# Bob-cheng/DepthModelHardening

Hardware: AMD Instinct MI355X
Metric: adv-train images/sec @1024x320, 10-step PGD, bs32 (higher is better)
Workload: dtype f32; 1 GPU; Monodepth2 ResNet18 1024x320, 10-step PGD-L_inf attack on 12 scenes, train batch 32/GPU, stereo photometric+SSIM+smoothness loss (md2), Adam; config_index=2, global_batch=32, per_gpu_batch=32, parallelism=dp1, attack_overlap=False, attack_scenes=12, graph_attack=False

## Files before the change

### depthmodelhardening_amd/csrc/down_conv.hip

```cpp
#include "common.hpp"

using namespace dmh;

namespace {

typedef float f32x16 __attribute__((ext_vector_type(16)));

constexpr int NT = 256;
constexpr int TR = 4, TC = 32;
constexpr int CK = 8, NPAIR = CK / 2;
constexpr unsigned OOB = 0x80000000u;

constexpr int A_PITCH = 36;
constexpr int A_ELEMS = 64 * 2 * A_PITCH;
constexpr int A_NW = A_ELEMS / NT;
constexpr int D_ELEMS = 64 * 2 * NPAIR;
constexpr int D_NW = D_ELEMS / NT;

template <int NW, int ND>
__device__ __forceinline__ void filter_offsets(int tid, int r0, int inner, unsigned (&wo)[NW], unsigned (&dofs)[ND]) {
#pragma unroll
    for (int i = 0; i < NW; ++i) {
        const int d = tid + i * NT, rowh = d / A_PITCH, q = d - rowh * A_PITCH;
        const int row = rowh >> 1, hh = rowh & 1, t = q >> 2, p = q & 3;
        wo[i] = (unsigned)(((r0 + row) * inner + 2 * p + hh) * 9 + t) * 4u;
    }
#pragma unroll
    for (int i = 0; i < ND; ++i) {
        const int d = tid + i * NT, rowh = d >> 2, p = d & 3;
        dofs[i] = (unsigned)((r0 + (rowh >> 1)) * inner + 2 * p + (rowh & 1)) * 4u;
    }
}

typedef float f32x4 __attribute__((ext_vector_type(4)));
constexpr int IMG_A = 32 * 2 * A_PITCH;
constexpr int IMG_D = 32 * 2 * NPAIR;
constexpr int IMG_G = IMG_A + IMG_D;
constexpr int IMG_WORDS = IMG_G / 4;
constexpr int IMG_NW = (IMG_WORDS + NT - 1) / NT;

__global__ __launch_bounds__(NT) void down_weight_image_kernel(const float* __restrict__ w3, const float* __restrict__ wd, int rows,
                                                               int inner, float* __restrict__ img) {
    const size_t idx = (size_t)blockIdx.x * NT + threadIdx.x;
    const int nch = inner / CK;
    if (idx >= (size_t)(rows / 32) * nch * IMG_G) return;
    const int e = (int)(idx % IMG_G);
    const int gc = (int)(idx / IMG_G), rg = gc / nch, ch = gc - rg * nch;
    float v;
    if (e < IMG_A) {
        const int rowh = e / A_PITCH, q = e - rowh * A_PITCH, t = q >> 2, p = q & 3;
        v = w3[((size_t)(rg * 32 + (rowh >> 1)) * inner + ch * CK + 2 * p + (rowh & 1)) * 9 + t];
    } else {
        const int d = e - IMG_A, rowh = d >> 2, p = d & 3;
        v = wd ? wd[(size_t)(rg * 32 + (rowh >> 1)) * inner + ch * CK + 2 * p + (rowh & 1)] : 0.f;
    }
    img[idx] = v;
}

__device__ __forceinline__ f32x4 ldb4(rsrc_t rs, unsigned byte_off, unsigned s_off) {
    return __builtin_bit_cast(f32x4, __builtin_amdgcn_raw_buffer_load_b128(rs, byte_off, s_off, 0));
}

constexpr int F_PR = 3 * TR, F_PC = 2 * TC + 1, F_PEL = F_PR * F_PC, F_PLANE = F_PEL + 1;
constexpr int F_NP = (CK * F_PEL + NT - 1) / NT;

struct FArgs {
    const float *x, *w3, *wd;
    const float *shift3, *shiftd;
    int relu3;
    float *y3, *yd;
    int B, Cin, Cout, H, W, Ho, Wo, gx, gy, gk;
};

template <bool DOWN>
__device__ __forceinline__ void fwd_store(const FArgs& a, const f32x16& accA, const f32x16& accB, const f32x16& accDA,
                                          const f32x16& accDB, int R, int ox, int h, int k0, int NR) {
    const int b = R / a.Ho, oy = R - b * a.Ho;
    if (R < NR && ox < a.Wo) {
        const size_t HWo = (size_t)a.Ho * a.Wo;
        const size_t o = ((size_t)b * a.Cout + k0) * HWo + (size_t)oy * a.Wo + ox;
#pragma unroll
        for (int v = 0; v < 16; ++v) {
            const int i = 8 * (v >> 2) + 4 * h + (v & 3);
            float ya = accA[v], yb = accB[v];
            if (a.shift3) {
                ya += a.shift3[k0 + i];
                yb += a.shift3[k0 + i + 32];
            }
            if (a.relu3) {
                ya = fmaxf(ya, 0.f);
                yb = fmaxf(yb, 0.f);
            }
            a.y3[o + (size_t)i * HWo] = ya;
            a.y3[o + (size_t)(i + 32) * HWo] = yb;
            if constexpr (DOWN) {
                float da = accDA[v], db = accDB[v];
                if (a.shiftd) {
                    da += a.shiftd[k0 + i];
                    db += a.shiftd[k0 + i + 32];
                }
                a.yd[o + (size_t)i * HWo] = da;
                a.yd[o + (size_t)(i + 32) * HWo] = db;
            }
        }
    }
}

template <bool DOWN>
__global__ __launch_bounds__(NT, 2) void down_conv_fwd_kernel(const FArgs a) {
    __shared__ float patch[CK * F_PLANE];
    __shared__ __attribute__((aligned(16))) float wt[A_ELEMS];
    __shared__ __attribute__((aligned(16))) float wdl[D_ELEMS];
    const int tid = threadIdx.x, lane = tid & 63, wv = tid >> 6, n = lane & 31, h = lane >> 5;
    int q = blockIdx.x;
    const int kt = q % a.gk;
    q /= a.gk;
    const int bxi = q % a.gx, rt = q / a.gx;
    const int R0 = rt * TR, ox0 = bxi * TC, k0 = kt * 64;
    const int ix0 = 2 * ox0 - 1, NR = a.B * a.Ho;
    const unsigned HW = (unsigned)(a.H * a.W);
    const rsrc_t rx = make_rsrc(a.x, (unsigned)a.B * (unsigned)a.Cin * HW * 4u);
    const rsrc_t rw = make_rsrc(a.w3, (unsigned)a.Cout * (unsigned)a.Cin * 36u);
    const rsrc_t rd = make_rsrc(DOWN ? a.wd : a.w3, (unsigned)a.Cout * (unsigned)a.Cin * 4u);

    unsigned po[F_NP], wo[A_NW], dofs[D_NW];
#pragma unroll
    for (int i = 0; i < F_NP; ++i) {
        const int e = tid + i * NT, c = e / F_PEL, rem = e - c * F_PEL, r = rem / F_PC, cc = rem - r * F_PC;
        const int R = R0 + r / 3, bb = R / a.Ho, oy = R - bb * a.Ho;
        const int iy = 2 * oy - 1 + r % 3, ix = ix0 + cc;
        const bool ok = e < CK * F_PEL && R < NR && iy >= 0 && iy < a.H && ix >= 0 && ix < a.W;
        po[i] = ok ? ((unsigned)(bb * a.Cin + c) * HW + (unsigned)(iy * a.W + ix)) * 4u : OOB;
    }
    filter_offsets(tid, k0, a.Cin, wo, dofs);

    float rp[F_NP], rwv[A_NW], rdv[D_NW];
    auto fetch = [&](const int c0) __attribute__((always_inline)) {
        const unsigned sp = (unsigned)c0 * HW * 4u, sw = (unsigned)c0 * 36u, sd = (unsigned)c0 * 4u;
#pragma unroll
        for (int i = 0; i < F_NP; ++i) rp[i] = ldb(rx, po[i], sp);
#pragma unroll
        for (int i = 0; i < A_NW; ++i) rwv[i] = ldb(rw, wo[i], sw);
        if constexpr (DOWN) {
#pragma unroll
            for (int i = 0; i < D_NW; ++i) rdv[i] = ldb(rd, dofs[i], sd);
        }
    };
    auto commit = [&]() __attribute__((always_inline)) {
#pragma unroll
        for (int i = 0; i < F_NP; ++i) {
            const int e = tid + i * NT;
            if (i < F_NP - 1 || e < CK * F_PEL) patch[e + e / F_PEL] = rp[i];
        }
#pragma unroll
        for (int i = 0; i < A_NW; ++i) wt[tid + i * NT] = rwv[i];
        if constexpr (DOWN) {
#pragma unroll
            for (int i = 0; i < D_NW; ++i) wdl[tid + i * NT] = rdv[i];
        }
    };

    f32x16 accA, accB, accDA, accDB;
#pragma unroll
    for (int v = 0; v < 16; ++v) accA[v] = accB[v] = accDA[v] = accDB[v] = 0.f;
    const float* pb = patch + h * F_PLANE + (3 * wv) * F_PC + 2 * n;
    const float* aA = wt + (n * 2 + h) * A_PITCH;
    const float* aB = aA + 32 * 2 * A_PITCH;
    const float* dA = wdl + (n * 2 + h) * NPAIR;
    const float* dB = dA + 32 * 2 * NPAIR;

    const int chunks = a.Cin / CK;
    fetch(0);
    for (int ch = 0; ch < chunks; ++ch) {
        __syncthreads();
        commit();
        __syncthreads();
        if (ch + 1 < chunks) fetch((ch + 1) * CK);
        float4 da = make_float4(0.f, 0.f, 0.f, 0.f), db = da;
        if constexpr (DOWN) {
            da = *reinterpret_cast<const float4*>(dA);
            db = *reinterpret_cast<const float4*>(dB);
        }
#pragma unroll
        for (int t = 0; t < 9; ++t) {
            const float4 wa = *reinterpret_cast<const float4*>(aA + 4 * t);
            const float4 wb = *reinterpret_cast<const float4*>(aB + 4 * t);
            const float was[4] = {wa.x, wa.y, wa.z, wa.w}, wbs[4] = {wb.x, wb.y, wb.z, wb.w};
            const float das[4] = {da.x, da.y, da.z, da.w}, dbs[4] = {db.x, db.y, db.z, db.w};
#pragma unroll
            for (int p = 0; p < NPAIR; ++p) {
                const float bv = pb[2 * p * F_PLANE + (t / 3) * F_PC + (t % 3)];
                accA = __builtin_amdgcn_mfma_f32_32x32x2f32(was[p], bv, accA, 0, 0, 0);
                accB = __builtin_amdgcn_mfma_f32_32x32x2f32(wbs[p], bv, accB, 0, 0, 0);
                if (DOWN && t == 4) {
                    accDA = __builtin_amdgcn_mfma_f32_32x32x2f32(das[p], bv, accDA, 0, 0, 0);
                    accDB = __builtin_amdgcn_mfma_f32_32x32x2f32(dbs[p], bv, accDB, 0, 0, 0);
                }
            }
        }
    }
    fwd_store<DOWN>(a, accA, accB, accDA, accDB, R0 + wv, ox0 + n, h, k0, NR);
}

constexpr int FW_WPR = 17, FW_SUB = 2 * FW_WPR, FW_ROW = 2 * FW_SUB;
constexpr int FW_PLANE = 864;
constexpr int FW_NWORD = CK * F_PR * FW_WPR;
constexpr int FW_NP = (FW_NWORD + NT - 1) / NT;
static_assert(FW_PLANE >= F_PR * FW_ROW && FW_PLANE % 64 == 32, "plane pitch");

template <bool DOWN>
__global__ __launch_bounds__(NT, 2) void down_conv_fwd_wide_kernel(const FArgs a) {
    __shared__ __attribute__((aligned(16))) float patch[CK * FW_PLANE];
    __shared__ f32x4 wimg[2 * IMG_WORDS];
    const int tid = threadIdx.x, lane = tid & 63, wv = tid >> 6, n = lane & 31, h = lane >> 5;
    int q = blockIdx.x;
    const int kt = q % a.gk;
    q /= a.gk;
    const int bxi = q % a.gx, rt = q / a.gx;
    const int R0 = rt * TR, ox0 = bxi * TC, k0 = kt * 64;
    const int NR = a.B * a.Ho, nch = a.Cin / CK;
    const unsigned HW = (unsigned)(a.H * a.W);
    const rsrc_t rx = make_rsrc(a.x, (unsigned)a.B * (unsigned)a.Cin * HW * 4u);
    const rsrc_t ri = make_rsrc(a.w3, (unsigned)(a.Cout / 32) * (unsigned)nch * (unsigned)(IMG_G * 4));

    unsigned po[FW_NP];
    int lo[FW_NP];
#pragma unroll
    for (int i = 0; i < FW_NP; ++i) {
        const int e = tid + i * NT, c = e / (F_PR * FW_WPR), rem = e - c * (F_PR * FW_WPR), r = rem / FW_WPR, w = rem - r * FW_WPR;
        const int R = R0 + r / 3, bb = R / a.Ho, oy = R - bb * a.Ho;
        const int iy = 2 * oy - 1 + r % 3, ix = 2 * ox0 - 4 + 4 * w;
        const bool ok = e < FW_NWORD && R < NR && iy >= 0 && iy < a.H && ix >= 0 && ix < a.W;
        po[i] = ok ? ((unsigned)(bb * a.Cin + c) * HW + (unsigned)(iy * a.W + ix)) * 4u : OOB;
        lo[i] = c * FW_PLANE + r * FW_ROW + 2 * w;
    }
    const unsigned wofs = (unsigned)tid * 16u;
    const unsigned gstep = (unsigned)nch * (unsigned)(IMG_G * 4);
    const unsigned g0 = (unsigned)(2 * kt) * gstep;

    f32x4 rp[FW_NP], rw[2 * IMG_NW];
    auto fetch = [&](const int ch) __attribute__((always_inline)) {
        const unsigned sp = (unsigned)(ch * CK) * HW * 4u;
#pragma unroll
        for (int i = 0; i < FW_NP; ++i) rp[i] = ldb4(rx, po[i], sp);
        const unsigned sw = g0 + (unsigned)ch * (unsigned)(IMG_G * 4);
#pragma unroll
        for (int g = 0; g < 2; ++g)
#pragma unroll
            for (int j = 0; j < IMG_NW; ++j)
                rw[g * IMG_NW + j] = ldb4(ri, ((j + 1) * NT <= IMG_WORDS || j * NT + tid < IMG_WORDS) ? wofs + (unsigned)(j * NT * 16) : OOB,
                                          sw + (unsigned)g * gstep);
    };
    auto commit = [&]() __attribute__((always_inline)) {
#pragma unroll
        for (int i = 0; i < FW_NP; ++i) {
            if (i < FW_NP - 1 || tid + i * NT < FW_NWORD) {
                *reinterpret_cast<float2*>(patch + lo[i]) = make_float2(rp[i][0], rp[i][2]);
                *reinterpret_cast<float2*>(patch + lo[i] + FW_SUB) = make_float2(rp[i][1], rp[i][3]);
            }
        }
#pragma unroll
        for (int g = 0; g < 2; ++g)
#pragma unroll
            for (int j = 0; j < IMG_NW; ++j)
                if ((j + 1) * NT <= IMG_WORDS || j * NT + tid < IMG_WORDS) wimg[g * IMG_WORDS + j * NT + tid] = rw[g * IMG_NW + j];
    };

    f32x16 accA, accB, accDA, accDB;
#pragma unroll
    for (int v = 0; v < 16; ++v) accA[v] = accB[v] = accDA[v] = accDB[v] = 0.f;
    const float* pb = patch + h * FW_PLANE + (3 * wv) * FW_ROW + n;
    const float* wf = reinterpret_cast<const float*>(wimg);
    const float* aA = wf + (n * 2 + h) * A_PITCH;
    const float* aB = aA + IMG_G;
    const float* dA = wf + IMG_A + (n * 2 + h) * NPAIR;
    const float* dB = dA + IMG_G;

    fetch(0);
    for (int ch = 0; ch < nch; ++ch) {
        __syncthreads();
        commit();
        __syncthreads();
        if (ch + 1 < nch) fetch(ch + 1);
        float4 da = make_float4(0.f, 0.f, 0.f, 0.f), db = da;
        if constexpr (DOWN) {
            da = *reinterpret_cast<const float4*>(dA);
            db = *reinterpret_cast<const float4*>(dB);
        }
#pragma unroll
        for (int t = 0; t < 9; ++t) {
            const float4 wa = *reinterpret_cast<const float4*>(aA + 4 * t);
            const float4 wb = *reinterpret_cast<const float4*>(aB + 4 * t);
            const float was[4] = {wa.x, wa.y, wa.z, wa.w}, wbs[4] = {wb.x, wb.y, wb.z, wb.w};
            const float das[4] = {da.x, da.y, da.z, da.w}, dbs[4] = {db.x, db.y, db.z, db.w};
            const int kx = t % 3, off = (t / 3) * FW_ROW + (kx == 1 ? 2 : FW_SUB + (kx == 0 ? 1 : 2));
#pragma unroll
            for (int p = 0; p < NPAIR; ++p) {
                const float bv = pb[2 * p * FW_PLANE + off];
                accA = __builtin_amdgcn_mfma_f32_32x32x2f32(was[p], bv, accA, 0, 0, 0);
                accB = __builtin_amdgcn_mfma_f32_32x32x2f32(wbs[p], bv, accB, 0, 0, 0);
                if (DOWN && t == 4) {
                    accDA = __builtin_amdgcn_mfma_f32_32x32x2f32(das[p], bv, accDA, 0, 0, 0);
                    accDB = __builtin_amdgcn_mfma_f32_32x32x2f32(dbs[p], bv, accDB, 0, 0, 0);
                }
            }
        }
    }
    fwd_store<DOWN>(a, accA, accB, accDA, accDB, R0 + wv, ox0 + n, h, k0, NR);
}

constexpr int B_PR = 2 * TR, B_PC = TC + 1, B_PEL = B_PR * B_PC, B_PLANE = B_PEL + 1;
constexpr int B_NP = (CK * B_PEL + NT - 1) / NT;
constexpr int G_PLANE = TR * TC + 1;
constexpr int G_NP = CK * TR * TC / NT;

struct BArgs {
    const float *g3, *gd, *w3t, *wdt;
    const float* gadd;
    float* gx;
    int B, Cin, Cout, H, W, Ho, Wo, tx, ty, gc;
};

template <int MH>
__device__ __forceinline__ void bwd_store(const BArgs& a, const f32x16 (&acc)[4][MH], int R, int bc, int h, int c0m, int NR) {
    const int b = R / a.Ho, ar = R - b * a.Ho;
    if (R < NR && bc < a.Wo) {
        const size_t HW = (size_t)a.H * a.W;
        const size_t o = ((size_t)b * a.Cin + c0m) * HW + (size_t)(2 * ar) * a.W + 2 * bc;
#pragma unroll
        for (int half = 0; half < MH; ++half)
#pragma unroll
            for (int v = 0; v < 16; ++v) {
                const int i = 8 * (v >> 2) + 4 * h + (v & 3) + 32 * half;
                float* g = a.gx + o + (size_t)i * HW;
                float2 r0 = make_float2(acc[0][half][v], acc[1][half][v]), r1 = make_float2(acc[2][half][v], acc[3][half][v]);
                if (a.gadd) {
                    const float* q = a.gadd + o + (size_t)i * HW;
                    const float2 q0 = *reinterpret_cast<const float2*>(q), q1 = *reinterpret_cast<const float2*>(q + a.W);
                    r0.x += q0.x; r0.y += q0.y; r1.x += q1.x; r1.y += q1.y;
                }
                *reinterpret_cast<float2*>(g) = r0;
                *reinterpret_cast<float2*>(g + a.W) = r1;
            }
    }
}

template <bool DOWN, int MH>
__global__ __launch_bounds__(NT, 2) void down_conv_bwd_kernel(const BArgs a) {
    constexpr int W_NW = A_NW * MH / 2, W_ND = D_NW * MH / 2;
    __shared__ float patch[CK * B_PLANE];
    __shared__ float gdl[CK * G_PLANE];
    __shared__ __attribute__((aligned(16))) float wt[A_ELEMS * MH / 2];
    __shared__ __attribute__((aligned(16))) float wdl[D_ELEMS * MH / 2];
    const int tid = threadIdx.x, lane = tid & 63, wv = tid >> 6, n = lane & 31, h = lane >> 5;
    int q = blockIdx.x;
    const int ct = q % a.gc;
    q /= a.gc;
    const int bxi = q % a.tx, rt = q / a.tx;
    const int R0 = rt * TR, b0 = bxi * TC, c0m = ct * 32 * MH, NR = a.B * a.Ho;
    const unsigned HWo = (unsigned)(a.Ho * a.Wo);
    const rsrc_t rg = make_rsrc(a.g3, (unsigned)a.B * (unsigned)a.Cout * HWo * 4u);
    const rsrc_t rgd = make_rsrc(DOWN ? a.gd : a.g3, (unsigned)a.B * (unsigned)a.Cout * HWo * 4u);
    const rsrc_t rw = make_rsrc(a.w3t, (unsigned)a.Cout * (unsigned)a.Cin * 36u);
    const rsrc_t rd = make_rsrc(DOWN ? a.wdt : a.w3t, (unsigned)a.Cout * (unsigned)a.Cin * 4u);

    unsigned po[B_NP], go[G_NP], wo[W_NW], dofs[W_ND];
#pragma unroll
    for (int i = 0; i < B_NP; ++i) {
        const int e = tid + i * NT, c = e / B_PEL, rem = e - c * B_PEL, r = rem / B_PC, cc = rem - r * B_PC;
        const int R = R0 + (r >> 1), bb = R / a.Ho, oy = R - bb * a.Ho + (r & 1), ox = b0 + cc;
        const bool ok = e < CK * B_PEL && R < NR && oy < a.Ho && ox < a.Wo;
        po[i] = ok ? ((unsigned)(bb * a.Cout + c) * HWo + (unsigned)(oy * a.Wo + ox)) * 4u : OOB;
    }
#pragma unroll
    for (int i = 0; i < G_NP; ++i) {
        const int e = tid + i * NT, c = e / (TR * TC), rem = e - c * (TR * TC), r = rem / TC, cc = rem - r * TC;
        const int R = R0 + r, bb = R / a.Ho, oy = R - bb * a.Ho, ox = b0 + cc;
        go[i] = (R < NR && ox < a.Wo) ? ((unsigned)(bb * a.Cout + c) * HWo + (unsigned)(oy * a.Wo + ox)) * 4u : OOB;
    }
    filter_offsets(tid, c0m, a.Cout, wo, dofs);

    float rp[B_NP], rg4[G_NP], rwv[W_NW], rdv[W_ND];
    auto fetch = [&](const int k0) __attribute__((always_inline)) {
        const unsigned sp = (unsigned)k0 * HWo * 4u, sw = (unsigned)k0 * 36u, sd = (unsigned)k0 * 4u;
#pragma unroll
        for (int i = 0; i < B_NP; ++i) rp[i] = ldb(rg, po[i], sp);
#pragma unroll
        for (int i = 0; i < W_NW; ++i) rwv[i] = ldb(rw, wo[i], sw);
        if constexpr (DOWN) {
#pragma unroll
            for (int i = 0; i < G_NP; ++i) rg4[i] = ldb(rgd, go[i], sp);
#pragma unroll
            for (int i = 0; i < W_ND; ++i) rdv[i] = ldb(rd, dofs[i], sd);
        }
    };
    auto commit = [&]() __attribute__((always_inline)) {
#pragma unroll
        for (int i = 0; i < B_NP; ++i) {
            const int e = tid + i * NT;
            if (i < B_NP - 1 || e < CK * B_PEL) patch[e + e / B_PEL] = rp[i];
        }
#pragma unroll
        for (int i = 0; i < W_NW; ++i) wt[tid + i * NT] = rwv[i];
        if constexpr (DOWN) {
#pragma unroll
            for (int i = 0; i < G_NP; ++i) {
                const int e = tid + i * NT, c = e / (TR * TC);
                gdl[e + c] = rg4[i];
            }
#pragma unroll
            for (int i = 0; i < W_ND; ++i) wdl[tid + i * NT] = rdv[i];
        }
    };

    f32x16 acc[4][MH];
#pragma unroll
    for (int c = 0; c < 4; ++c)
#pragma unroll
        for (int m = 0; m < MH; ++m)
#pragma unroll
            for (int v = 0; v < 16; ++v) acc[c][m][v] = 0.f;
    const float* pg = patch + h * B_PLANE + (2 * wv) * B_PC + n;
    const float* pd = gdl + h * G_PLANE + wv * TC + n;
    const float* aA = wt + (n * 2 + h) * A_PITCH;
    const float* aB = aA + 32 * 2 * A_PITCH;
    const float* dA = wdl + (n * 2 + h) * NPAIR;
    const float* dB = dA + 32 * 2 * NPAIR;

    const int chunks = a.Cout / CK;
    fetch(0);
    for (int ch = 0; ch < chunks; ++ch) {
        __syncthreads();
        commit();
        __syncthreads();
        if (ch + 1 < chunks) fetch((ch + 1) * CK);
        float bv[NPAIR][2][2];
#pragma unroll
        for (int p = 0; p < NPAIR; ++p) {
            bv[p][0][0] = pg[2 * p * B_PLANE];
            bv[p][0][1] = pg[2 * p * B_PLANE + 1];
            bv[p][1][0] = pg[2 * p * B_PLANE + B_PC];
            bv[p][1][1] = pg[2 * p * B_PLANE + B_PC + 1];
        }
#pragma unroll
        for (int t = 0; t < 9; ++t) {
            const int ky = t / 3, kx = t % 3;
            const int cls = 2 * (ky != 1 ? 1 : 0) + (kx != 1 ? 1 : 0), dy = ky == 0 ? 1 : 0, dx = kx == 0 ? 1 : 0;
            const float4 wa = *reinterpret_cast<const float4*>(aA + 4 * t);
            const float4 wb = *reinterpret_cast<const float4*>((MH == 2 ? aB : aA) + 4 * t);
            const float was[4] = {wa.x, wa.y, wa.z, wa.w}, wbs[4] = {wb.x, wb.y, wb.z, wb.w};
#pragma unroll
            for (int p = 0; p < NPAIR; ++p) {
                acc[cls][0] = __builtin_amdgcn_mfma_f32_32x32x2f32(was[p], bv[p][dy][dx], acc[cls][0], 0, 0, 0);
                if constexpr (MH == 2)
                    acc[cls][1] = __builtin_amdgcn_mfma_f32_32x32x2f32(wbs[p], bv[p][dy][dx], acc[cls][1], 0, 0, 0);
            }
        }
        if constexpr (DOWN) {
            const float4 da = *reinterpret_cast<const float4*>(dA), db = *reinterpret_cast<const float4*>(MH == 2 ? dB : dA);
            const float das[4] = {da.x, da.y, da.z, da.w}, dbs[4] = {db.x, db.y, db.z, db.w};
#pragma unroll
            for (int p = 0; p < NPAIR; ++p) {
                const float gv = pd[2 * p * G_PLANE];
                acc[0][0] = __builtin_amdgcn_mfma_f32_32x32x2f32(das[p], gv, acc[0][0], 0, 0, 0);
                if constexpr (MH == 2) acc[0][1] = __builtin_amdgcn_mfma_f32_32x32x2f32(dbs[p], gv, acc[0][1], 0, 0, 0);
            }
        }
    }
    bwd_store<MH>(a, acc, R0 + wv, b0 + n, h, c0m, NR);
}

constexpr int BW_WPR = 9, BW_ROW = 4 * BW_WPR, BW_PLANE = B_PR * BW_ROW;
constexpr int BW_NWORD = CK * B_PR * BW_WPR;
constexpr int BW_NP = (BW_NWORD + NT - 1) / NT;
constexpr int GW_PLANE = 160;
static_assert(BW_PLANE % 64 == 32 && GW_PLANE % 64 == 32 && CK * TR * (TC / 4) == NT, "wide backward layout");

template <bool DOWN, int MH>
__global__ __launch_bounds__(NT, 2) void down_conv_bwd_wide_kernel(const BArgs a) {
    __shared__ f32x4 patch4[CK * BW_PLANE / 4];
    __shared__ f32x4 gdl4[CK * GW_PLANE / 4];
    __shared__ f32x4 wimg[MH * IMG_WORDS];
    const int tid = threadIdx.x, lane = tid & 63, wv = tid >> 6, n = lane & 31, h = lane >> 5;
    int q = blockIdx.x;
    const int ct = q % a.gc;
    q /= a.gc;
    const int bxi = q % a.tx, rt = q / a.tx;
    const int R0 = rt * TR, b0 = bxi * TC, c0m = ct * 32 * MH, NR = a.B * a.Ho, nch = a.Cout / CK;
    const unsigned HWo = (unsigned)(a.Ho * a.Wo);
    const rsrc_t rg = make_rsrc(a.g3, (unsigned)a.B * (unsigned)a.Cout * HWo * 4u);
    const rsrc_t rgd = make_rsrc(DOWN ? a.gd : a.g3, (unsigned)a.B * (unsigned)a.Cout * HWo * 4u);
    const rsrc_t ri = make_rsrc(a.w3t, (unsigned)(a.Cin / 32) * (unsigned)nch * (unsigned)(IMG_G * 4));

    unsigned po[BW_NP], go;
#pragma unroll
    for (int i = 0; i < BW_NP; ++i) {
        const int e = tid + i * NT, c = e / (B_PR * BW_WPR), rem = e - c * (B_PR * BW_WPR), r = rem / BW_WPR, w = rem - r * BW_WPR;
        const int R = R0 + (r >> 1), bb = R / a.Ho, oy = R - bb * a.Ho + (r & 1), ox = b0 + 4 * w;
        const bool ok = e < BW_NWORD && R < NR && oy < a.Ho && ox < a.Wo;
        po[i] = ok ? ((unsigned)(bb * a.Cout + c) * HWo + (unsigned)(oy * a.Wo + ox)) * 4u : OOB;
    }
    {
        const int c = tid / (TR * (TC / 4)), rem = tid - c * (TR * (TC / 4)), r = rem / (TC / 4), w = rem - r * (TC / 4);
        const int R = R0 + r, bb = R / a.Ho, oy = R - bb * a.Ho, ox = b0 + 4 * w;
        go = (R < NR && ox < a.Wo) ? ((unsigned)(bb * a.Cout + c) * HWo + (unsigned)(oy * a.Wo + ox)) * 4u : OOB;
    }
    const int gslot = (tid / (TR * (TC / 4))) * (GW_PLANE / 4) + (tid % (TR * (TC / 4)));
    const unsigned wofs = (unsigned)tid * 16u;
    const unsigned gstep = (unsigned)nch * (unsigned)(IMG_G * 4);
    const unsigned g0 = (unsigned)(ct * MH) * gstep;

    f32x4 rp[BW_NP], rg4, rw[MH * IMG_NW];
    auto fetch = [&](const int ch) __attribute__((always_inline)) {
        const unsigned sp = (unsigned)(ch * CK) * HWo * 4u;
#pragma unroll
        for (int i = 0; i < BW_NP; ++i) rp[i] = ldb4(rg, po[i], sp);
        if constexpr (DOWN) rg4 = ldb4(rgd, go, sp);
        const unsigned sw = g0 + (unsigned)ch * (unsigned)(IMG_G * 4);
#pragma unroll
        for (int g = 0; g < MH; ++g)
#pragma unroll
            for (int j = 0; j < IMG_NW; ++j)
                rw[g * IMG_NW + j] = ldb4(ri, ((j + 1) * NT <= IMG_WORDS || j * NT + tid < IMG_WORDS) ? wofs + (unsigned)(j * NT * 16) : OOB,
                                          sw + (unsigned)g * gstep);
    };
    auto commit = [&]() __attribute__((always_inline)) {
#pragma unroll
        for (int i = 0; i < BW_NP; ++i)
            if ((i + 1) * NT <= BW_NWORD || tid + i * NT < BW_NWORD) patch4[tid + i * NT] = rp[i];
        if constexpr (DOWN) gdl4[gslot] = rg4;
#pragma unroll
        for (int g = 0; g < MH; ++g)
#pragma unroll
            for (int j = 0; j < IMG_NW; ++j)
                if ((j + 1) * NT <= IMG_WORDS || j * NT + tid < IMG_WORDS) wimg[g * IMG_WORDS + j * NT + tid] = rw[g * IMG_NW + j];
    };

    f32x16 acc[4][MH];
#pragma unroll
    for (int c = 0; c < 4; ++c)
#pragma unroll
        for (int m = 0; m < MH; ++m)
#pragma unroll
            for (int v = 0; v < 16; ++v) acc[c][m][v] = 0.f;
    const float* pg = reinterpret_cast<const float*>(patch4) + h * BW_PLANE + (2 * wv) * BW_ROW + n;
    const float* pd = reinterpret_cast<const float*>(gdl4) + h * GW_PLANE + wv * TC + n;
    const float* wf = reinterpret_cast<const float*>(wimg);
    const float* aA = wf + (n * 2 + h) * A_PITCH;
    const float* aB = aA + (MH == 2 ? IMG_G : 0);
    const float* dA = wf + IMG_A + (n * 2 + h) * NPAIR;
    const float* dB = dA + (MH == 2 ? IMG_G : 0);

    fetch(0);
    for (int ch = 0; ch < nch; ++ch) {
        __syncthreads();
        commit();
        __syncthreads();
        if (ch + 1 < nch) fetch(ch + 1);
        float bv[NPAIR][2][2];
#pragma unroll
        for (int p = 0; p < NPAIR; ++p) {
            bv[p][0][0] = pg[2 * p * BW_PLANE];
            bv[p][0][1] = pg[2 * p * BW_PLANE + 1];
            bv[p][1][0] = pg[2 * p * BW_PLANE + BW_ROW];
            bv[p][1][1] = pg[2 * p * BW_PLANE + BW_ROW + 1];
        }
#pragma unroll
        for (int t = 0; t < 9; ++t) {
            const int ky = t / 3, kx = t % 3;
            const int cls = 2 * (ky != 1 ? 1 : 0) + (kx != 1 ? 1 : 0), dy = ky == 0 ? 1 : 0, dx = kx == 0 ? 1 : 0;
            const float4 wa = *reinterpret_cast<const float4*>(aA + 4 * t);
            const float4 wb = *reinterpret_cast<const float4*>(aB + 4 * t);
            const float was[4] = {wa.x, wa.y, wa.z, wa.w}, wbs[4] = {wb.x, wb.y, wb.z, wb.w};
#pragma unroll
            for (int p = 0; p < NPAIR; ++p) {
                acc[cls][0] = __builtin_amdgcn_mfma_f32_32x32x2f32(was[p], bv[p][dy][dx], acc[cls][0], 0, 0, 0);
                if constexpr (MH == 2)
                    acc[cls][1] = __builtin_amdgcn_mfma_f32_32x32x2f32(wbs[p], bv[p][dy][dx], acc[cls][1], 0, 0, 0);
            }
        }
        if constexpr (DOWN) {
            const float4 da = *reinterpret_cast<const float4*>(dA), db = *reinterpret_cast<const float4*>(dB);
            const float das[4] = {da.x, da.y, da.z, da.w}, dbs[4] = {db.x, db.y, db.z, db.w};
#pragma unroll
            for (int p = 0; p < NPAIR; ++p) {
                const float gv = pd[2 * p * GW_PLANE];
                acc[0][0] = __builtin_amdgcn_mfma_f32_32x32x2f32(das[p], gv, acc[0][0], 0, 0, 0);
                if constexpr (MH == 2) acc[0][1] = __builtin_amdgcn_mfma_f32_32x32x2f32(dbs[p], gv, acc[0][1], 0, 0, 0);
            }
        }
    }
    bwd_store<MH>(a, acc, R0 + wv, b0 + n, h, c0m, NR);
}

int check_sizes(int B, int Cin, int Cout, int H, int W) {
    DMH_REQUIRE(B > 0 && Cin > 0 && Cout > 0 && H >= 2 && W >= 2 && (H & 1) == 0 && (W & 1) == 0,
                "input height and width must be even");
    const int64_t cmax = Cin > Cout ? Cin : Cout;
    DMH_REQUIRE((int64_t)B * cmax * H * W < ((int64_t)1 << 29) && (int64_t)Cin * Cout < ((int64_t)1 << 24),
                "tensor too large (32-bit byte offsets)");
    return DMH_OK;
}

}

extern "C" {

int dmh_down_conv_fwd_act(const float* x, const float* w3, const float* wd, const float* shift3, const float* shiftd,
                          int relu3, int B, int Cin, int Cout, int H, int W, float* y3, float* yd, void* stream);

int dmh_down_conv_fwd(const float* x, const float* w3, const float* wd, int B, int Cin, int Cout, int H, int W,
                      float* y3, float* yd, void* stream) {
    return dmh_down_conv_fwd_act(x, w3, wd, nullptr, nullptr, 0, B, Cin, Cout, H, W, y3, yd, stream);
}

int dmh_down_conv_fwd_act(const float* x, const float* w3, const float* wd, const float* shift3, const float* shiftd,
                          int relu3, int B, int Cin, int Cout, int H, int W, float* y3, float* yd, void* stream) {
    DMH_REQUIRE(x && w3 && y3 && ((wd == nullptr) == (yd == nullptr)), "null pointer");
    DMH_REQUIRE(shiftd == nullptr || wd != nullptr, "shiftd without the shortcut convolution");
    if (int rc = check_sizes(B, Cin, Cout, H, W)) return rc;
    DMH_REQUIRE(Cin % CK == 0 && Cout % 64 == 0, "C_in must be a multiple of 8 and C_out of 64");
    FArgs a;
    a.x = x;
    a.w3 = w3;
    a.wd = wd;
    a.shift3 = shift3;
    a.shiftd = shiftd;
    a.relu3 = relu3 ? 1 : 0;
    a.y3 = y3;
    a.yd = yd;
    a.B = B;
    a.Cin = Cin;
    a.Cout = Cout;
    a.H = H;
    a.W = W;
    a.Ho = H / 2;
    a.Wo = W / 2;
    a.gx = (a.Wo + TC - 1) / TC;
    a.gy = (B * a.Ho + TR - 1) / TR;
    a.gk = Cout / 64;
    const long long blocks = (long long)a.gx * a.gy * a.gk;
    DMH_REQUIRE(blocks < (1ll << 31), "grid too large");
    if (wd)
        hipLaunchKernelGGL(down_conv_fwd_kernel<true>, dim3((unsigned)blocks), dim3(NT), 0, (hipStream_t)stream, a);
    else
        hipLaunchKernelGGL(down_conv_fwd_kernel<false>, dim3((unsigned)blocks), dim3(NT), 0, (hipStream_t)stream, a);
    return check_launch("dmh_down_conv_fwd_act");
}

int64_t dmh_down_conv_image_size(int rows, int inner) {
    if (rows <= 0 || inner <= 0 || rows % 32 || inner % CK) return -1;
    return (int64_t)(rows / 32) * (inner / CK) * IMG_G;
}

int dmh_down_conv_weight_image(const float* w3, const float* wd, int rows, int inner, float* image, void* stream) {
    DMH_REQUIRE(w3 && image, "null pointer");
    const int64_t n = dmh_down_conv_image_size(rows, inner);
    DMH_REQUIRE(n > 0 && n < ((int64_t)1 << 29), "rows must be a multiple of 32 and inner of 8");
    hipLaunchKernelGGL(down_weight_image_kernel, dim3((unsigned)((n + NT - 1) / NT)), dim3(NT), 0, (hipStream_t)stream, w3, wd, rows,
                       inner, image);
    return check_launch("dmh_down_conv_weight_image");
}

int dmh_down_conv_fwd_img(const float* x, const float* image, int has_down, const float* shift3, const float* shiftd, int relu3,
                          int B, int Cin, int Cout, int H, int W, float* y3, float* yd, void* stream) {
    DMH_REQUIRE(x && image && y3 && ((has_down != 0) == (yd != nullptr)), "null pointer");
    DMH_REQUIRE(shiftd == nullptr || has_down, "shiftd without the shortcut convolution");
    if (int rc = check_sizes(B, Cin, Cout, H, W)) return rc;
    DMH_REQUIRE(Cin % CK == 0 && Cout % 64 == 0, "C_in must be a multiple of 8 and C_out of 64");
    DMH_REQUIRE(W % 4 == 0, "the image form reads 16-byte words: W must be a multiple of 4 (use dmh_down_conv_fwd_act otherwise)");
    FArgs a;
    a.x = x;
    a.w3 = image;
    a.wd = has_down ? image : nullptr;
    a.shift3 = shift3;
    a.shiftd = shiftd;
    a.relu3 = relu3 ? 1 : 0;
    a.y3 = y3;
    a.yd = yd;
    a.B = B;
    a.Cin = Cin;
    a.Cout = Cout;
    a.H = H;
    a.W = W;
    a.Ho = H / 2;
    a.Wo = W / 2;
    a.gx = (a.Wo + TC - 1) / TC;
    a.gy = (B * a.Ho + TR - 1) / TR;
    a.gk = Cout / 64;
    const long long blocks = (long long)a.gx * a.gy * a.gk;
    DMH_REQUIRE(blocks < (1ll << 31), "grid too large");
    if (has_down)
        hipLaunchKernelGGL(down_conv_fwd_wide_kernel<true>, dim3((unsigned)blocks), dim3(NT), 0, (hipStream_t)stream, a);
    else
        hipLaunchKernelGGL(down_conv_fwd_wide_kernel<false>, dim3((unsigned)blocks), dim3(NT), 0, (hipStream_t)stream, a);
    return check_launch("dmh_down_conv_fwd_img");
}

int dmh_down_conv_bwd_data(const float* g3, const float* gd, const float* w3t, const float* wdt, int B, int Cin, int Cout,
                           int H, int W, float* g_x, void* stream) {
    return dmh_down_conv_bwd_data_acc(g3, gd, w3t, wdt, nullptr, B, Cin, Cout, H, W, g_x, stream);
}

int dmh_down_conv_bwd_data_acc(const float* g3, const float* gd, const float* w3t, const float* wdt, const float* g_add, int B,
                               int Cin, int Cout, int H, int W, float* g_x, void* stream) {
    DMH_REQUIRE(g3 && w3t && g_x && ((gd == nullptr) == (wdt == nullptr)), "null pointer");
    if (int rc = check_sizes(B, Cin, Cout, H, W)) return rc;
    DMH_REQUIRE(Cout % CK == 0 && Cin % 64 == 0, "C_out must be a multiple of 8 and C_in of 64");
    const long long tiles = (long long)((W / 2 + TC - 1) / TC) * ((B * (H / 2) + TR - 1) / TR);
    const int mh = tiles * (Cin / 64) < 200 ? 1 : 2;
    BArgs a;
    a.g3 = g3;
    a.gd = gd;
    a.w3t = w3t;
    a.wdt = wdt;
    a.gadd = g_add;
    a.gx = g_x;
    a.B = B;
    a.Cin = Cin;
    a.Cout = Cout;
    a.H = H;
    a.W = W;
    a.Ho = H / 2;
    a.Wo = W / 2;
    a.tx = (a.Wo + TC - 1) / TC;
    a.ty = (B * a.Ho + TR - 1) / TR;
    a.gc = Cin / (32 * mh);
    const long long blocks = (long long)a.tx * a.ty * a.gc;
    DMH_REQUIRE(blocks < (1ll << 31), "grid too large");
    if (gd && mh == 2)
        hipLaunchKernelGGL((down_conv_bwd_kernel<true, 2>), dim3((unsigned)blocks), dim3(NT), 0, (hipStream_t)stream, a);
    else if (gd)
        hipLaunchKernelGGL((down_conv_bwd_kernel<true, 1>), dim3((unsigned)blocks), dim3(NT), 0, (hipStream_t)stream, a);
    else if (mh == 2)
        hipLaunchKernelGGL((down_conv_bwd_kernel<false, 2>), dim3((unsigned)blocks), dim3(NT), 0, (hipStream_t)stream, a);
    else
        hipLaunchKernelGGL((down_conv_bwd_kernel<false, 1>), dim3((unsigned)blocks), dim3(NT), 0, (hipStream_t)stream, a);
    return check_launch("dmh_down_conv_bwd_data");
}

int dmh_down_conv_bwd_data_img(const float* g3, const float* gd, const float* image, const float* g_add, int B, int Cin, int Cout,
                               int H, int W, float* g_x, void* stream) {
    DMH_REQUIRE(g3 && image && g_x, "null pointer");
    if (int rc = check_sizes(B, Cin, Cout, H, W)) return rc;
    DMH_REQUIRE(Cout % CK == 0 && Cin % 64 == 0, "C_out must be a multiple of 8 and C_in of 64");
    DMH_REQUIRE(W % 8 == 0, "the image form reads 16-byte words: W must be a multiple of 8 (use dmh_down_conv_bwd_data_acc otherwise)");
    const long long tiles = (long long)((W / 2 + TC - 1) / TC) * ((B * (H / 2) + TR - 1) / TR);
    const int mh = tiles * (Cin / 64) < 200 ? 1 : 2;
    BArgs a;
    a.g3 = g3;
    a.gd = gd;
    a.w3t = image;
    a.wdt = gd ? image : nullptr;
    a.gadd = g_add;
    a.gx = g_x;
    a.B = B;
    a.Cin = Cin;
    a.Cout = Cout;
    a.H = H;
    a.W = W;
    a.Ho = H / 2;
    a.Wo = W / 2;
    a.tx = (a.Wo + TC - 1) / TC;
    a.ty = (B * a.Ho + TR - 1) / TR;
    a.gc = Cin / (32 * mh);
    const long long blocks = (long long)a.tx * a.ty * a.gc;
    DMH_REQUIRE(blocks < (1ll << 31), "grid too large");
    if (gd && mh == 2)
        hipLaunchKernelGGL((down_conv_bwd_wide_kernel<true, 2>), dim3((unsigned)blocks), dim3(NT), 0, (hipStream_t)stream, a);
    else if (gd)
        hipLaunchKernelGGL((down_conv_bwd_wide_kernel<true, 1>), dim3((unsigned)blocks), dim3(NT), 0, (hipStream_t)stream, a);
    else if (mh == 2)
        hipLaunchKernelGGL((down_conv_bwd_wide_kernel<false, 2>), dim3((unsigned)blocks), dim3(NT), 0, (hipStream_t)stream, a);
    else
        hipLaunchKernelGGL((down_conv_bwd_wide_kernel<false, 1>), dim3((unsigned)blocks), dim3(NT), 0, (hipStream_t)stream, a);
    return check_launch("dmh_down_conv_bwd_data_img");
}

}
```

Baseline: 405.6 images/s.

## Add double-buffered LDS pipelined kernels for strided down-conv forward and backward

Adds new forward and backward-data kernels for the stride-2 down convolution that double-buffer input tiles and weight images in dynamic LDS. The global loads for chunk ch+2 are interleaved with the MFMA issue of chunk ch under explicit scheduling barriers, so memory latency is hidden behind compute. The forward pipe kernel is used only when the grid fits within one wave of CUs, while the backward pipe kernel is always used. The larger LDS footprint may reduce occupancy, and the register staging adds pressure.

```diff
diff --git a/depthmodelhardening_amd/csrc/down_conv.hip b/depthmodelhardening_amd/csrc/down_conv.hip
--- a/depthmodelhardening_amd/csrc/down_conv.hip
+++ b/depthmodelhardening_amd/csrc/down_conv.hip
@@ -591,6 +591,335 @@
         }
     }
     bwd_store<MH>(a, acc, R0 + wv, b0 + n, h, c0m, NR);
+}
+
+#ifndef DMH_DOWN_PIPE
+#define DMH_DOWN_PIPE 1
+#endif
+constexpr int IMGP_WORDS = IMG_NW * NT;
+constexpr unsigned RSRC_FLAGS = 0x00020000;
+
+__device__ __forceinline__ rsrc_t rsrc_sized(const void* p, unsigned bytes) {
+    return __builtin_amdgcn_make_buffer_rsrc(const_cast<void*>(p), 0, bytes, RSRC_FLAGS);
+}
+__device__ __forceinline__ void pipe_barrier() {
+    asm volatile("s_waitcnt lgkmcnt(0)" ::: "memory");
+    __builtin_amdgcn_s_barrier();
+    asm volatile("" ::: "memory");
+}
+
+constexpr int FP_WIMG = CK * FW_PLANE;
+constexpr int FP_BUF = FP_WIMG + 2 * IMGP_WORDS * 4;
+constexpr int FP_PAD = F_PR * FW_ROW;
+constexpr size_t FP_SMEM = 2 * FP_BUF * sizeof(float);
+constexpr int FP_UNITS = FW_NP + 2 * IMG_NW;
+static_assert(FP_PAD + FW_SUB + 2 <= FW_PLANE && FP_WIMG % 4 == 0 && FP_BUF % 4 == 0, "forward pipeline layout");
+
+template <bool DOWN>
+__global__ __launch_bounds__(NT) void down_conv_fwd_pipe_kernel(const FArgs a) {
+    extern __shared__ f32x4 smem[];
+    float* const lds = reinterpret_cast<float*>(smem);
+    const int tid = threadIdx.x, lane = tid & 63, wv = tid >> 6, n = lane & 31, h = lane >> 5;
+    int q = blockIdx.x;
+    const int kt = q % a.gk;
+    q /= a.gk;
+    const int bxi = q % a.gx, rt = q / a.gx;
+    const int R0 = rt * TR, ox0 = bxi * TC, k0 = kt * 64;
+    const int NR = a.B * a.Ho, nch = a.Cin / CK;
+    const unsigned HW = (unsigned)(a.H * a.W);
+    const unsigned xbytes = (unsigned)a.B * (unsigned)a.Cin * HW * 4u;
+    const unsigned ibytes = (unsigned)(a.Cout / 32) * (unsigned)nch * (unsigned)(IMG_G * 4);
+
+    unsigned po[FW_NP], wo[IMG_NW];
+    int lo[FW_NP];
+#pragma unroll
+    for (int i = 0; i < FW_NP; ++i) {
+        const int e = tid + i * NT, c = e / (F_PR * FW_WPR), rem = e - c * (F_PR * FW_WPR), r = rem / FW_WPR, w = rem - r * FW_WPR;
+        const int R = R0 + r / 3, bb = R / a.Ho, oy = R - bb * a.Ho;
+        const int iy = 2 * oy - 1 + r % 3, ix = 2 * ox0 - 4 + 4 * w;
+        const bool ok = e < FW_NWORD && R < NR && iy >= 0 && iy < a.H && ix >= 0 && ix < a.W;
+        po[i] = ok ? ((unsigned)(bb * a.Cin + c) * HW + (unsigned)(iy * a.W + ix)) * 4u : OOB;
+        lo[i] = e < FW_NWORD ? c * FW_PLANE + r * FW_ROW + 2 * w : FP_PAD;
+    }
+#pragma unroll
+    for (int j = 0; j < IMG_NW; ++j) wo[j] = j * NT + tid < IMG_WORDS ? (unsigned)(j * NT + tid) * 16u : OOB;
+    const unsigned gstep = (unsigned)nch * (unsigned)(IMG_G * 4);
+    const unsigned g0 = (unsigned)(2 * kt) * gstep;
+
+    f32x4 rp[FW_NP], rw[2 * IMG_NW];
+    auto put = [&](const int k, float* nb) __attribute__((always_inline)) {
+        if (k < FW_NP) {
+            *reinterpret_cast<float2*>(nb + lo[k]) = make_float2(rp[k][0], rp[k][2]);
+            *reinterpret_cast<float2*>(nb + lo[k] + FW_SUB) = make_float2(rp[k][1], rp[k][3]);
+        } else {
+            const int g = (k - FW_NP) / IMG_NW, j = (k - FW_NP) % IMG_NW;
+            reinterpret_cast<f32x4*>(nb + FP_WIMG)[g * IMGP_WORDS + j * NT + tid] = rw[k - FW_NP];
+        }
+    };
+    auto get = [&](const int k, const rsrc_t rxs, const rsrc_t ris, const int ch) __attribute__((always_inline)) {
+        if (k < FW_NP) {
+            rp[k] = ldb4(rxs, po[k], (unsigned)(ch * CK) * HW * 4u);
+        } else {
+            const int g = (k - FW_NP) / IMG_NW, j = (k - FW_NP) % IMG_NW;
+            rw[k - FW_NP] = ldb4(ris, wo[j], g0 + (unsigned)ch * (unsigned)(IMG_G * 4) + (unsigned)g * gstep);
+        }
+    };
+
+    f32x16 accA, accB, accDA, accDB;
+#pragma unroll
+    for (int v = 0; v < 16; ++v) accA[v] = accB[v] = accDA[v] = accDB[v] = 0.f;
+    const int pbo = h * FW_PLANE + (3 * wv) * FW_ROW + n;
+    const int aAo = FP_WIMG + (n * 2 + h) * A_PITCH, aBo = aAo + IMGP_WORDS * 4;
+    const int dAo = FP_WIMG + IMG_A + (n * 2 + h) * NPAIR, dBo = dAo + IMGP_WORDS * 4;
+
+    {
+        const rsrc_t rx = rsrc_sized(a.x, xbytes), ri = rsrc_sized(a.w3, ibytes);
+        const rsrc_t rx1 = rsrc_sized(a.x, nch > 1 ? xbytes : 0u), ri1 = rsrc_sized(a.w3, nch > 1 ? ibytes : 0u);
+#pragma unroll
+        for (int k = 0; k < FP_UNITS; ++k) get(k, rx, ri, 0);
+#pragma unroll
+        for (int k = 0; k < FP_UNITS; ++k) {
+            put(k, lds);
+            get(k, rx1, ri1, 1);
+        }
+        pipe_barrier();
+    }
+    for (int ch = 0; ch < nch; ++ch) {
+        const int cur = ch & 1;
+        const float* cb = lds + cur * FP_BUF;
+        float* nb = lds + (cur ^ 1) * FP_BUF;
+        const bool more = ch + 2 < nch;
+        const rsrc_t rxs = rsrc_sized(a.x, more ? xbytes : 0u), ris = rsrc_sized(a.w3, more ? ibytes : 0u);
+        const float* pb = cb + pbo;
+        float4 wa[2], wb[2], da = make_float4(0.f, 0.f, 0.f, 0.f), db = da;
+        float bv[2][NPAIR];
+        wa[0] = *reinterpret_cast<const float4*>(cb + aAo);
+        wb[0] = *reinterpret_cast<const float4*>(cb + aBo);
+#pragma unroll
+        for (int p = 0; p < NPAIR; ++p) bv[0][p] = pb[2 * p * FW_PLANE + FW_SUB + 1];
+        __builtin_amdgcn_sched_barrier(0);
+#pragma unroll
+        for (int t = 0; t < 9; ++t) {
+            const int tb = t & 1;
+            const float was[4] = {wa[tb].x, wa[tb].y, wa[tb].z, wa[tb].w}, wbs[4] = {wb[tb].x, wb[tb].y, wb[tb].z, wb[tb].w};
+            const float das[4] = {da.x, da.y, da.z, da.w}, dbs[4] = {db.x, db.y, db.z, db.w};
+            const int tn = t + 1, kxn = tn % 3, offn = (tn / 3) * FW_ROW + (kxn == 1 ? 2 : FW_SUB + (kxn == 0 ? 1 : 2));
+#pragma unroll
+            for (int p = 0; p < NPAIR; ++p) {
+                const int s = 4 * t + p;
+                const float b = bv[tb][p];
+                accA = __builtin_amdgcn_mfma_f32_32x32x2f32(was[p], b, accA, 0, 0, 0);
+                accB = __builtin_amdgcn_mfma_f32_32x32x2f32(wbs[p], b, accB, 0, 0, 0);
+                if (DOWN && t == 4) {
+                    accDA = __builtin_amdgcn_mfma_f32_32x32x2f32(das[p], b, accDA, 0, 0, 0);
+                    accDB = __builtin_amdgcn_mfma_f32_32x32x2f32(dbs[p], b, accDB, 0, 0, 0);
+                }
+                if (t < 8) {
+                    if (p == 0) {
+                        wa[tb ^ 1] = *reinterpret_cast<const float4*>(cb + aAo + 4 * tn);
+                        wb[tb ^ 1] = *reinterpret_cast<const float4*>(cb + aBo + 4 * tn);
+                    }
+                    bv[tb ^ 1][p] = pb[2 * p * FW_PLANE + offn];
+                }
+                if (DOWN && s == 1) {
+                    da = *reinterpret_cast<const float4*>(cb + dAo);
+                    db = *reinterpret_cast<const float4*>(cb + dBo);
+                }
+                if (s >= 4 && (s & 1) == 0 && (s - 4) / 2 < FP_UNITS) {
+                    put((s - 4) / 2, nb);
+                    get((s - 4) / 2, rxs, ris, ch + 2);
+                }
+                __builtin_amdgcn_sched_barrier(0);
+            }
+        }
+        pipe_barrier();
+    }
+    fwd_store<DOWN>(a, accA, accB, accDA, accDB, R0 + wv, ox0 + n, h, k0, NR);
+}
+
+constexpr int BP_GDL = CK * BW_PLANE / 4, BP_WIMG = BP_GDL + CK * GW_PLANE / 4;
+constexpr int BP_PAD = BP_GDL + TR * TC / 4;
+static_assert(TR * TC + 4 <= GW_PLANE && BW_NP == 3 && (BW_NP - 1) * NT <= BW_NWORD, "backward pipeline layout");
+
+template <bool DOWN, int MH>
+__global__ __launch_bounds__(NT, 2) void down_conv_bwd_pipe_kernel(const BArgs a) {
+    constexpr int BUFW = BP_WIMG + MH * IMGP_WORDS;
+    constexpr int NG = DOWN ? 1 : 0, UNITS = BW_NP + NG + MH * IMG_NW;
+    extern __shared__ f32x4 smem[];
+    const int tid = threadIdx.x, lane = tid & 63, wv = tid >> 6, n = lane & 31, h = lane >> 5;
+    int q = blockIdx.x;
+    const int ct = q % a.gc;
+    q /= a.gc;
+    const int bxi = q % a.tx, rt = q / a.tx;
+    const int R0 = rt * TR, b0 = bxi * TC, c0m = ct * 32 * MH, NR = a.B * a.Ho, nch = a.Cout / CK;
+    const unsigned HWo = (unsigned)(a.Ho * a.Wo);
+    const unsigned gbytes = (unsigned)a.B * (unsigned)a.Cout * HWo * 4u;
+    const unsigned ibytes = (unsigned)(a.Cin / 32) * (unsigned)nch * (unsigned)(IMG_G * 4);
+    const float* const gdp = DOWN ? a.gd : a.g3;
+
+    unsigned po[BW_NP], go, wo[IMG_NW];
+#pragma unroll
+    for (int i = 0; i < BW_NP; ++i) {
+        const int e = tid + i * NT, c = e / (B_PR * BW_WPR), rem = e - c * (B_PR * BW_WPR), r = rem / BW_WPR, w = rem - r * BW_WPR;
+        const int R = R0 + (r >> 1), bb = R / a.Ho, oy = R - bb * a.Ho + (r & 1), ox = b0 + 4 * w;
+        const bool ok = e < BW_NWORD && R < NR && oy < a.Ho && ox < a.Wo;
+        po[i] = ok ? ((unsigned)(bb * a.Cout + c) * HWo + (unsigned)(oy * a.Wo + ox)) * 4u : OOB;
+    }
+    {
+        const int c = tid / (TR * (TC / 4)), rem = tid - c * (TR * (TC / 4)), r = rem / (TC / 4), w = rem - r * (TC / 4);
+        const int R = R0 + r, bb = R / a.Ho, oy = R - bb * a.Ho, ox = b0 + 4 * w;
+        go = (R < NR && ox < a.Wo) ? ((unsigned)(bb * a.Cout + c) * HWo + (unsigned)(oy * a.Wo + ox)) * 4u : OOB;
+    }
+#pragma unroll
+    for (int j = 0; j < IMG_NW; ++j) wo[j] = j * NT + tid < IMG_WORDS ? (unsigned)(j * NT + tid) * 16u : OOB;
+    const int gslot = BP_GDL + (tid / (TR * (TC / 4))) * (GW_PLANE / 4) + (tid % (TR * (TC / 4)));
+    const int plast = tid + (BW_NP - 1) * NT < BW_NWORD ? tid + (BW_NP - 1) * NT : BP_PAD;
+    const unsigned gstep = (unsigned)nch * (unsigned)(IMG_G * 4);
+    const unsigned g0 = (unsigned)(ct * MH) * gstep;
+
+    f32x4 rp[BW_NP], rg4, rw[MH * IMG_NW];
+    auto put = [&](const int k, f32x4* nb) __attribute__((always_inline)) {
+        if (k < BW_NP - 1) nb[tid + k * NT] = rp[k];
+        else if (k == BW_NP - 1) nb[plast] = rp[k];
+        else if (k < BW_NP + NG) nb[gslot] = rg4;
+        else {
+            const int g = (k - BW_NP - NG) / IMG_NW, j = (k - BW_NP - NG) % IMG_NW;
+            nb[BP_WIMG + g * IMGP_WORDS + j * NT + tid] = rw[k - BW_NP - NG];
+        }
+    };
+    auto get = [&](const int k, const rsrc_t rgs, const rsrc_t rds, const rsrc_t ris, const int ch) __attribute__((always_inline)) {
+        const unsigned sp = (unsigned)(ch * CK) * HWo * 4u;
+        if (k < BW_NP) rp[k] = ldb4(rgs, po[k], sp);
+        else if (k < BW_NP + NG) rg4 = ldb4(rds, go, sp);
+        else {
+            const int g = (k - BW_NP - NG) / IMG_NW, j = (k - BW_NP - NG) % IMG_NW;
+            rw[k - BW_NP - NG] = ldb4(ris, wo[j], g0 + (unsigned)ch * (unsigned)(IMG_G * 4) + (unsigned)g * gstep);
+        }
+    };
+
+    f32x16 acc[4][MH];
+#pragma unroll
+    for (int c = 0; c < 4; ++c)
+#pragma unroll
+        for (int m = 0; m < MH; ++m)
+#pragma unroll
+            for (int v = 0; v < 16; ++v) acc[c][m][v] = 0.f;
+    const int pgo = h * BW_PLANE + (2 * wv) * BW_ROW + n;
+    const int pdo = BP_GDL * 4 + h * GW_PLANE + wv * TC + n;
+    const int aAo = BP_WIMG * 4 + (n * 2 + h) * A_PITCH, aBo = aAo + (MH == 2 ? IMGP_WORDS * 4 : 0);
+    const int dAo = BP_WIMG * 4 + IMG_A + (n * 2 + h) * NPAIR, dBo = dAo + (MH == 2 ? IMGP_WORDS * 4 : 0);
+
+    {
+        const rsrc_t rg = rsrc_sized(a.g3, gbytes), rd = rsrc_sized(gdp, gbytes), ri = rsrc_sized(a.w3t, ibytes);
+        const unsigned gb1 = nch > 1 ? gbytes : 0u;
+        const rsrc_t rg1 = rsrc_sized(a.g3, gb1), rd1 = rsrc_sized(gdp, gb1), ri1 = rsrc_sized(a.w3t, nch > 1 ? ibytes : 0u);
+#pragma unroll
+        for (int k = 0; k < UNITS; ++k) get(k, rg, rd, ri, 0);
+#pragma unroll
+        for (int k = 0; k < UNITS; ++k) {
+            put(k, smem);
+            get(k, rg1, rd1, ri1, 1);
+        }
+        pipe_barrier();
+    }
+    for (int ch = 0; ch < nch; ++ch) {
+        const int cur = ch & 1;
+        const float* cb = reinterpret_cast<const float*>(smem + cur * BUFW);
+        f32x4* nb = smem + (cur ^ 1) * BUFW;
+        const bool more = ch + 2 < nch;
+        const unsigned gbs = more ? gbytes : 0u;
+        const rsrc_t rgs = rsrc_sized(a.g3, gbs), rds = rsrc_sized(gdp, gbs), ris = rsrc_sized(a.w3t, more ? ibytes : 0u);
+        const float* pg = cb + pgo;
+        float bv[NPAIR][2][2];
+        float4 wa[2], wb[2];
+        float gv[NPAIR] = {0.f, 0.f, 0.f, 0.f};
+        auto read_bv = [&](const int p) __attribute__((always_inline)) {
+            bv[p][0][0] = pg[2 * p * BW_PLANE];
+            bv[p][0][1] = pg[2 * p * BW_PLANE + 1];
+            bv[p][1][0] = pg[2 * p * BW_PLANE + BW_ROW];
+            bv[p][1][1] = pg[2 * p * BW_PLANE + BW_ROW + 1];
+        };
+        read_bv(0);
+        wa[0] = *reinterpret_cast<const float4*>(cb + aAo);
+        wb[0] = *reinterpret_cast<const float4*>(cb + aBo);
+#pragma unroll
+        for (int p = 1; p < NPAIR; ++p) read_bv(p);
+        __builtin_amdgcn_sched_barrier(0);
+#pragma unroll
+        for (int t = 0; t < 9; ++t) {
+            const int ky = t / 3, kx = t % 3, tb = t & 1;
+            const int cls = 2 * (ky != 1 ? 1 : 0) + (kx != 1 ? 1 : 0), dy = ky == 0 ? 1 : 0, dx = kx == 0 ? 1 : 0;
+            const float was[4] = {wa[tb].x, wa[tb].y, wa[tb].z, wa[tb].w}, wbs[4] = {wb[tb].x, wb[tb].y, wb[tb].z, wb[tb].w};
+#pragma unroll
+            for (int p = 0; p < NPAIR; ++p) {
+                const int s = 4 * t + p;
+                acc[cls][0] = __builtin_amdgcn_mfma_f32_32x32x2f32(was[p], bv[p][dy][dx], acc[cls][0], 0, 0, 0);
+                if constexpr (MH == 2)
+                    acc[cls][1] = __builtin_amdgcn_mfma_f32_32x32x2f32(wbs[p], bv[p][dy][dx], acc[cls][1], 0, 0, 0);
+                if (p == 0 && (t < 8 || DOWN)) {
+                    wa[tb ^ 1] = *reinterpret_cast<const float4*>(cb + (t < 8 ? aAo + 4 * (t + 1) : dAo));
+                    wb[tb ^ 1] = *reinterpret_cast<const float4*>(cb + (t < 8 ? aBo + 4 * (t + 1) : dBo));
+                }
+                if (DOWN && t == 8) gv[p] = cb[pdo + 2 * p * GW_PLANE];
+                if (s >= 3 && s % 3 == 0 && s / 3 - 1 < UNITS) {
+                    put(s / 3 - 1, nb);
+                    get(s / 3 - 1, rgs, rds, ris, ch + 2);
+                }
+                __builtin_amdgcn_sched_barrier(0);
+            }
+        }
+        if constexpr (DOWN) {
+            const float das[4] = {wa[1].x, wa[1].y, wa[1].z, wa[1].w}, dbs[4] = {wb[1].x, wb[1].y, wb[1].z, wb[1].w};
+#pragma unroll
+            for (int p = 0; p < NPAIR; ++p) {
+                acc[0][0] = __builtin_amdgcn_mfma_f32_32x32x2f32(das[p], gv[p], acc[0][0], 0, 0, 0);
+                if constexpr (MH == 2) acc[0][1] = __builtin_amdgcn_mfma_f32_32x32x2f32(dbs[p], gv[p], acc[0][1], 0, 0, 0);
+            }
+        }
+        pipe_barrier();
+    }
+    bwd_store<MH>(a, acc, R0 + wv, b0 + n, h, c0m, NR);
+}
+
+int num_cus() {
+    static int n = 0;
+    if (n == 0) {
+        int dev = 0;
+        if (hipGetDevice(&dev) != hipSuccess ||
+            hipDeviceGetAttribute(&n, hipDeviceAttributeMultiprocessorCount, dev) != hipSuccess || n <= 0)
+            n = 256;
+    }
+    return n;
+}
+
+template <bool DOWN>
+int launch_fwd_pipe(const FArgs& a, unsigned blocks, hipStream_t st) {
+    static std::atomic<uint64_t> configured{0};
+    if (configure_dynamic_lds(down_conv_fwd_pipe_kernel<DOWN>, FP_SMEM, configured) != hipSuccess)
+        return fail(DMH_ELAUNCH, "%s: cannot raise the dynamic LDS limit", "dmh_down_conv_fwd_img");
+    hipLaunchKernelGGL(down_conv_fwd_pipe_kernel<DOWN>, dim3(blocks), dim3(NT), FP_SMEM, st, a);
+    return check_launch("dmh_down_conv_fwd_img");
+}
+
+template <bool DOWN, int MH>
+int launch_bwd_pipe(const BArgs& a, unsigned blocks, hipStream_t st) {
+    constexpr size_t smem = 2 * (size_t)(BP_WIMG + MH * IMGP_WORDS) * sizeof(f32x4);
+    static std::atomic<uint64_t> configured{0};
+    if (configure_dynamic_lds(down_conv_bwd_pipe_kernel<DOWN, MH>, smem, configured) != hipSuccess)
+        return fail(DMH_ELAUNCH, "%s: cannot raise the dynamic LDS limit", "dmh_down_conv_bwd_data_img");
+    hipLaunchKernelGGL((down_conv_bwd_pipe_kernel<DOWN, MH>), dim3(blocks), dim3(NT), smem, st, a);
+    return check_launch("dmh_down_conv_bwd_data_img");
+}
+
+bool fwd_pipe(long long blocks) {
+#if DMH_DOWN_PIPE == 1
+    return blocks <= num_cus();
+#else
+    return DMH_DOWN_PIPE != 0;
+#endif
+}
+bool bwd_pipe(long long blocks) {
+    return DMH_DOWN_PIPE != 0;
 }
 
 int check_sizes(int B, int Cin, int Cout, int H, int W) {
@@ -690,6 +1019,9 @@
     a.gk = Cout / 64;
     const long long blocks = (long long)a.gx * a.gy * a.gk;
     DMH_REQUIRE(blocks < (1ll << 31), "grid too large");
+    if (fwd_pipe(blocks))
+        return has_down ? launch_fwd_pipe<true>(a, (unsigned)blocks, (hipStream_t)stream)
+                        : launch_fwd_pipe<false>(a, (unsigned)blocks, (hipStream_t)stream);
     if (has_down)
         hipLaunchKernelGGL(down_conv_fwd_wide_kernel<true>, dim3((unsigned)blocks), dim3(NT), 0, (hipStream_t)stream, a);
     else
@@ -766,6 +1098,11 @@
     a.gc = Cin / (32 * mh);
     const long long blocks = (long long)a.tx * a.ty * a.gc;
     DMH_REQUIRE(blocks < (1ll << 31), "grid too large");
+    if (bwd_pipe(blocks)) {
+        hipStream_t st = (hipStream_t)stream;
+        if (gd) return mh == 2 ? launch_bwd_pipe<true, 2>(a, (unsigned)blocks, st) : launch_bwd_pipe<true, 1>(a, (unsigned)blocks, st);
+        return mh == 2 ? launch_bwd_pipe<false, 2>(a, (unsigned)blocks, st) : launch_bwd_pipe<false, 1>(a, (unsigned)blocks, st);
+    }
     if (gd && mh == 2)
         hipLaunchKernelGGL((down_conv_bwd_wide_kernel<true, 2>), dim3((unsigned)blocks), dim3(NT), 0, (hipStream_t)stream, a);
     else if (gd)
```

After: 407.7 images/s, median of 6. About the same (+0.5%).
